# Nyrox/raymond

Measured on AMD Instinct MI355X. Metric: Msamples/s (whole node) + achieved HBM GB/s, 1920x1080 @ 500spp 5-bounce, higher is better.
Workload: dtype f64

## Files before the change

include/raymond_hip_probe.h:

```cpp
#ifndef RAYMOND_HIP_PROBE_H
#define RAYMOND_HIP_PROBE_H

#include "raymond_hip.h"

#ifdef __cplusplus
extern "C" {
#endif

rmd_status rmd_probe_philox4x32_10(rmd_context *ctx, size_t n, const uint32_t *ctr4, const uint32_t *key2, uint32_t *out4);
rmd_status rmd_probe_block_uniforms(rmd_context *ctx, uint64_t seed, size_t n, const uint32_t *pixel, const uint32_t *sample,
                                    const uint32_t *block, double *out5);
rmd_status rmd_probe_sphere_intersect(rmd_context *ctx, size_t n, const double *sphere4, const double *ray6, int32_t *hit, double *t);
rmd_status rmd_probe_sphere_normal(rmd_context *ctx, size_t n, const double *sphere4, const double *ray6, const double *t, double *n3);
rmd_status rmd_probe_plane_intersect(rmd_context *ctx, size_t n, const double *plane6, const double *ray6, int32_t *hit, double *t);
rmd_status rmd_probe_aabb_intersect(rmd_context *ctx, size_t n, const double *aabb6, const double *ray6, int32_t *hit, double *t);
rmd_status rmd_probe_triangle_intersect(rmd_context *ctx, size_t n, const double *pos9, const double *ray6, int32_t *hit, double *t);
rmd_status rmd_probe_triangle_normal(rmd_context *ctx, size_t n, const double *pos9, const double *nrm9, const double *ray6,
                                     const double *t, double *n3);
rmd_status rmd_probe_onb(rmd_context *ctx, size_t n, const double *n3, double *t3, double *b3);
rmd_status rmd_probe_cosine_hemisphere(rmd_context *ctx, size_t n, const double *r1, const double *r2, double *dir3, double *pdf);
rmd_status rmd_probe_importance_sample_ggx(rmd_context *ctx, size_t n, const double *reflect3, const double *rough, const double *r1,
                                           const double *r2, double *dir3);
rmd_status rmd_probe_ggx_distribution(rmd_context *ctx, size_t n, const double *n3, const double *h3, const double *rough, double *out);
rmd_status rmd_probe_geometry_smith(rmd_context *ctx, size_t n, const double *n3, const double *v3, const double *l3,
// ... 1 lines not shown
rmd_status rmd_probe_fresnel_schlick(rmd_context *ctx, size_t n, const double *cos_theta, const double *f0_3, double *out3);
rmd_status rmd_probe_elementary(rmd_context *ctx, size_t n, const double *x, double *sqrt_out, double *sin_out, double *cos_out,
                                double *root_out, double *inv_root_out);
rmd_status rmd_probe_primary_ray(rmd_context *ctx, size_t n, const rmd_camera *cam, const uint32_t *xy2, const double *u2, double *ray6);
rmd_status rmd_probe_scene_intersect(rmd_context *ctx, const rmd_scene *scene, size_t n, const double *ray6, int32_t *obj, double *t,
                                     uint32_t *sub);
rmd_status rmd_probe_grid_intersect(rmd_context *ctx, const rmd_scene *scene, uint32_t g, size_t n, const double *ray6, int32_t *hit,
                                    double *t, uint32_t *tri);
rmd_status rmd_probe_grid_intersect_deep(rmd_context *ctx, const rmd_scene *scene, uint32_t g, size_t n, const double *ray6, uint32_t cut_lanes,
                                         uint32_t cut_round, uint32_t rays_per_wave, int32_t *hit, double *t, uint32_t *tri);
rmd_status rmd_probe_trace_samples(rmd_context *ctx, const rmd_scene *scene, const rmd_camera *cam, const rmd_settings *settings,
                                   size_t n, const uint32_t *xy2, const uint32_t *sample, double *rgb_out, int32_t *path_obj,
                                   uint32_t *path_sub);

rmd_status rmd_probe_triangle_sphere(size_t n, const double *pos9, double *out5);
rmd_status rmd_probe_launch_plan(uint32_t mode, uint32_t grid, size_t n, const uint32_t *in5, uint64_t *out8);
rmd_status rmd_probe_launch_sizes(uint32_t mode, uint32_t grid, uint64_t *out8);
rmd_status rmd_probe_scene_layout(const rmd_scene *scene, uint32_t *n_objects, uint32_t *n_grids, uint32_t *mask_words_total);
rmd_status rmd_probe_pretest_pairs(rmd_context *ctx, size_t n, const double *sphere5, const double *pos9, const double *ray6, int32_t *pass,
                                   int32_t *hit, double *t);

#ifdef __cplusplus
}
#endif
#endif
```

raymond_amd/csrc/api.cpp:

```cpp
#define RMD_WITH_HIP 1
#include <algorithm>
#include <cmath>
#include <limits>
#include <cstdio>
#include <cstdlib>
#include <cstring>
#include <new>

#include "internal.hpp"
#include "launch.hpp"

namespace {
thread_local std::string tl_last_error;

rmd_status bind(rmd_context *ctx) {
	if (!ctx) return rmd::fail(nullptr, RMD_ERR_INVALID_ARGUMENT, "null context");
	RMD_HIP(ctx, hipSetDevice(ctx->device));
	return RMD_OK;
}

rmd_status context_create(int32_t device, hipStream_t stream, bool own_stream, rmd_context **out) {
	if (!out) return rmd::fail(nullptr, RMD_ERR_INVALID_ARGUMENT, "rmd_context_create: null out pointer");
	*out = nullptr;
	int count = 0;
// ... 137 lines not shown
	f[0] = 0u, f[1] = 0u, f[2] = 0u;
	std::string what;
	if (code & kFaultTripLoop) what += " trip loop of render_wave;";
	if (code & kFaultSortedTripLoop) what += " trip loop of render_wave_sorted;";
	if (code & kFaultWorkLoop) what += " work loop of a persistent workgroup;";
	if (code & kFaultWalkRounds) what += " round loop of a grid walk;";
	if (code & kFaultQueuedTripLoop) what += " trip loop of render_wave_queued;";
	if (code & ~(kFaultTripLoop | kFaultSortedTripLoop | kFaultWorkLoop | kFaultWalkRounds | kFaultQueuedTripLoop)) what += " unknown code;";
	char num[96];
	std::snprintf(num, sizeof(num), " %u wave(s) reported, the last one at work item %u (code 0x%x)", reports, item, code);
	return fail(ctx, RMD_ERR_DEVICE_FAULT,
	            "device fault: a loop of the render kernel ran past its bound —" + what + num +
	                "; the launch was cut short and the framebuffer it wrote to is not valid");
}

RenderParams make_params(const rmd_context *ctx, const rmd_scene *scene, const rmd_camera *cam, const rmd_settings *st) {
	const double PI = 3.14159265358979323846;
	RenderParams P;
	std::memset(&P, 0, sizeof(P));
	for (int a = 0; a < 3; a++) P.cam_pos[a] = cam->position[a];
	P.width = (double)cam->backbuffer_width;
	P.height = (double)cam->backbuffer_height;
	P.inv_width = rmd::exact_reciprocal(P.width), P.inv_height = rmd::exact_reciprocal(P.height);
	P.aspect = P.width / P.height;
	P.tan_half_fov = std::tan(cam->fov_vert / 2.0 * PI / 180.0);
	P.focal_length = cam->focal_length;
	P.aperture_radius = cam->aperture_radius;
	P.W = cam->backbuffer_width, P.H = cam->backbuffer_height;
	P.bounce_limit = st->bounce_limit;
	P.sample_begin = st->sample_begin, P.sample_count = st->sample_count;
	P.n_objects = scene ? scene->n_objects : 0;
	P.n_grids = scene ? scene->n_grids : 0;
	P.mask_words_total = scene ? scene->mask_words_total : 0;
	P.key0 = (uint32_t)st->seed, P.key1 = (uint32_t)(st->seed >> 32);
	P.use_dof = ((st->flags & RMD_RENDER_DOF) && cam->aperture_radius > 0.0) ? 1u : 0u;
	P.end_black_paths = (st->flags & RMD_RENDER_TRACE_BLACK_PATHS) ? 0u : ((st->flags & RMD_RENDER_END_BLACK_PATHS) || !scene || (scene->n_grids == 0u && scene->regular)) ? 1u : 0u;
	P.shade_last_depth = (scene && !scene->regular) ? 1u : 0u;
	P.axis_pairs = scene ? scene->axis_pairs : 0u;
	P.visit_mask = scene ? scene->visit_mask : ~0ull, P.grid_mask = scene ? scene->grid_mask : ~0ull;
	P.fault = ctx ? ctx->d_fault : nullptr;
	P.walk_batch = rmd::kWalkBatchDefault;
	if (ctx && ctx->tunable[RMD_TUNE_WALK_BATCH] > 0) P.walk_batch = (uint32_t)ctx->tunable[RMD_TUNE_WALK_BATCH];
	{
		uint32_t k = rmd::kWalkCutDefault;
		if (ctx && ctx->tunable[RMD_TUNE_WALK_CUT] > 0) k = (uint32_t)std::min<int64_t>(ctx->tunable[RMD_TUNE_WALK_CUT] - 1, 31);
		P.walk_cut = (scene && scene->n_grid_objects == 1u) ? (k | (2u * k) << 8) : 0u;
		P.walk_steps_bound = scene ? scene->walk_steps_bound : 0u;
	}
#if RMD_DIAG
	if (ctx) P.debug_flags = ctx->debug_flags;
#endif
	return P;
}

// ... 116 lines not shown
			}
		}
		out.aux.assign((size_t)g.n_tris * 4, 0.0);
		for (uint64_t ti = 0; ti < g.n_tris; ti++) rmd::triangle_aux(g.tri_pos + (size_t)ti * 9, out.aux.data() + (size_t)ti * 4);
		out.spheres.assign((size_t)g.n_tris * 4, 0.0);
		out.sphere_kb = 0.0;
		for (uint64_t ti = 0; ti < g.n_tris; ti++) {
			double kb = 0.0;
			rmd::triangle_sphere(g.tri_pos + (size_t)ti * 9, out.spheres.data() + (size_t)ti * 4, kb);
			out.sphere_kb = std::max(out.sphere_kb, kb);
		}
	}
	return RMD_OK;
}

static rmd_status scene_create_impl(rmd_context *ctx, const rmd_object *objects, uint32_t n_objects, const rmd_grid_desc *grids, uint32_t n_grids,
                                    rmd_scene **out) {
	if (rmd_status s = bind(ctx)) return s;
	if (!out || (n_objects && !objects) || (n_grids && !grids)) return rmd::fail(ctx, RMD_ERR_INVALID_ARGUMENT, "rmd_scene_create: null argument");
	std::vector<rmd::DevObject> hobj(n_objects);
	bool regular = true;
	for (uint32_t i = 0; i < n_objects; i++) {
		const rmd_object &o = objects[i];
		rmd::DevObject &d = hobj[i];
		std::memset(&d, 0, sizeof(d));
		if (o.geometry_kind > RMD_GEOM_GRID) return rmd::fail(ctx, RMD_ERR_INVALID_ARGUMENT, "rmd_scene_create: unknown geometry kind");
		if (o.material.kind > RMD_MAT_EMISSION) return rmd::fail(ctx, RMD_ERR_INVALID_ARGUMENT, "rmd_scene_create: unknown material kind");
		if (o.geometry_kind == RMD_GEOM_GRID && o.grid_index >= n_grids) return rmd::fail(ctx, RMD_ERR_INVALID_ARGUMENT, "rmd_scene_create: grid_index out of range");
		d.geometry_kind = o.geometry_kind, d.grid_index = o.grid_index, d.material_kind = o.material.kind;
		for (int a = 0; a < 3; a++) d.origin[a] = o.origin[a], d.normal[a] = o.normal[a], d.color[a] = o.material.color[a];
		d.radius = o.radius;
		if (o.material.kind != RMD_MAT_EMISSION && std::fabs(o.material.roughness) > rmd::kMaxRoughness)
			return rmd::fail(ctx, RMD_ERR_UNSUPPORTED, "rmd_scene_create: |roughness| > 512 is not supported");
		if (o.material.kind != RMD_MAT_EMISSION && o.material.roughness != 0.0 && std::fabs(o.material.roughness) < rmd::kMinRoughness)
			return rmd::fail(ctx, RMD_ERR_UNSUPPORTED, "rmd_scene_create: 0 < |roughness| < 1e-12 is not supported");
// ... 13 lines not shown
		}
		if (o.material.kind == RMD_MAT_DIFFUSE && o.material.color[0] == 0.0 && o.material.color[1] == 0.0 && o.material.color[2] == 0.0) d.flags |= rmd::kObjBlackDiffuse;
	}
	for (uint32_t j = 0; j < n_objects; j++) {
		if (hobj[j].geometry_kind != RMD_GEOM_PLANE) continue;
		for (uint32_t i = 0; i < j; i++) {
			if (hobj[i].geometry_kind != RMD_GEOM_PLANE || hobj[i].pair_info != 0u) continue;
			bool opposite = true;
			for (int a = 0; a < 3; a++) opposite = opposite && hobj[j].normal[a] == -hobj[i].normal[a];
			if (!opposite) continue;
			hobj[i].pair_info = rmd::kPairTestedAtPartner | j, hobj[j].pair_info = i + 1u;
			break;
		}
	}
	uint32_t axis_pairs = 0;
	for (uint32_t j = 0; j < n_objects && j < 1023u && regular && ctx->tunable[RMD_TUNE_AXIS_PAIRS] != 1; j++) {
		if (hobj[j].geometry_kind != RMD_GEOM_PLANE || hobj[j].pair_info == 0u || (hobj[j].pair_info & rmd::kPairTestedAtPartner)) continue;
		const uint32_t i = hobj[j].pair_info - 1u;
		int k = -1, nonzero = 0;
		for (int a = 0; a < 3; a++)
			if (hobj[i].normal[a] != 0.0) nonzero++, k = a;
		if (nonzero != 1 || (hobj[i].normal[k] != 1.0 && hobj[i].normal[k] != -1.0) || ((axis_pairs >> (10 * k)) & 1023u) != 0u) continue;
		axis_pairs |= (j + 1u) << (10 * k);
		hobj[j].flags |= rmd::kObjAxisPair | ((uint32_t)k << rmd::kObjAxisShift) | (hobj[i].normal[k] == 1.0 ? rmd::kObjAxisEarlierIsPlus : 0u);
		hobj[i].flags |= rmd::kObjAxisPair;
		hobj[j].partner_origin_k = hobj[i].origin[k];
		hobj[j].pair_info = rmd::kPairTestedAtPartner | rmd::kPairAxis | i;
		hobj[i].pair_info |= rmd::kPairAxis;
	}
	auto sc = std::make_unique<rmd_scene>();
	sc->ctx = ctx, sc->n_objects = n_objects, sc->n_grids = n_grids, sc->regular = regular;
	sc->axis_pairs = axis_pairs;
	rmd::DevObject walls_block;
	std::memset(&walls_block, 0, sizeof(walls_block));
	{
		rmd::AxisWalls walls[3];
		std::memset(walls, 0, sizeof(walls));
		for (int k = 0; k < 3; k++) {
			const uint32_t f = (axis_pairs >> (10 * k)) & 1023u;
			if (f == 0u) continue;
			const uint32_t j = f - 1u, i = hobj[j].pair_info & 0x3FFFFFFFu;
			const bool e_plus = (hobj[j].flags & rmd::kObjAxisEarlierIsPlus) != 0u;
			walls[k].o_plus = e_plus ? hobj[i].origin[k] : hobj[j].origin[k], walls[k].o_minus = e_plus ? hobj[j].origin[k] : hobj[i].origin[k];
			walls[k].idx_plus = e_plus ? i : j, walls[k].idx_minus = e_plus ? j : i;
		}
		std::memcpy(&walls_block, walls, sizeof(walls));
	}
	sc->visit_mask = 0ull, sc->grid_mask = 0ull;
	for (uint32_t i = 0; i < n_objects && i < 64u; i++) {
		if (!(hobj[i].geometry_kind == RMD_GEOM_PLANE && (hobj[i].pair_info & rmd::kPairTestedAtPartner))) sc->visit_mask |= 1ull << i;
		if (hobj[i].geometry_kind == RMD_GEOM_GRID) sc->grid_mask |= 1ull << i;
	}
	for (uint32_t i = 0; i < n_objects; i++) sc->n_grid_objects += objects[i].geometry_kind == RMD_GEOM_GRID ? 1u : 0u;
	auto upload = [&](const void *src, size_t bytes, void **dst) -> hipError_t {
		*dst = nullptr;
		rmd::DeviceBuffer b;
		hipError_t e = b.alloc(bytes ? bytes : 16);
		if (e != hipSuccess) return e;
		*dst = b.as<void>();
		sc->owned.push_back(std::move(b));
		if (bytes) e = hipMemcpy(*dst, src, bytes, hipMemcpyHostToDevice);
		return e;
	};
	std::vector<rmd::DevGrid> hgrid(n_grids);
	for (uint32_t gi = 0; gi < n_grids; gi++) {
		const rmd_grid_desc &g = grids[gi];
		rmd::DevGrid &d = hgrid[gi];
// ... 261 lines not shown
		if ((P.debug_flags & 16u) && ctx->last_launch.queued) {
			static const char *kinds[3] = {"GEN  ", "SHADE", "WALK "};
			for (int k = 0; k < 3; k++)
				std::fprintf(stderr, "[rmd queued stamps, cycles] %s trips=%llu fetch=%llu make_ray=%llu simple=%llu walk=%llu ray_push=%llu classify=%llu stores=%llu\n", kinds[k], h[k * 8 + 7],
				             h[k * 8 + 0], h[k * 8 + 1], h[k * 8 + 2], h[k * 8 + 3], h[k * 8 + 4], h[k * 8 + 5], h[k * 8 + 6]);
			std::fprintf(stderr, "[rmd queued stamps, cycles] inside the walks: init=%llu stepping=%llu entry_wait=%llu scan=%llu (chunk search+load+test)=%llu hits=%llu tail=%llu\n",
			             h[24], h[25], h[26], h[27], h[29], h[30], h[31]);
		} else if (P.debug_flags & 16u)
			std::fprintf(stderr, "[rmd stamps, cycles] wave_total=%llu next_ray=%llu simple=%llu walk=%llu classify=%llu | walk: init=%llu stepping=%llu entry_wait=%llu scan=%llu (chunk search+load+test)=%llu hits=%llu tail=%llu\n",
			             h[0], h[1], h[2], h[3], h[4], h[8], h[9], h[10], h[11], h[13], h[14], h[15]);
		else
			std::fprintf(stderr, "[rmd debug] walk_calls=%llu walkers=%llu calls_with_walkers=%llu rounds=%llu wave_steps=%llu lane_steps=%llu test_rounds=%llu tests=%llu chunks=%llu | main_iterations=%llu live_lanes=%llu lanes_with_ray=%llu | stepping iterations with <= 4 / 8 / 16 lanes: %llu / %llu / %llu, with <= 8 lanes while tests wait: %llu\n",
			             h[0], h[1], h[2], h[3], h[4], h[5], h[6], h[8], h[9], h[10], h[11], h[12], h[7], h[13], h[14], h[15]);
		if ((P.debug_flags & 16u) == 0u)
			std::fprintf(stderr, "[rmd debug] sphere pre-test: pairs passed=%llu full chunks=%llu | pairs dropped that pass the reference's test (flag 64; must be 0)=%llu\n", h[17], h[18], h[16]);
		if ((P.debug_flags & 16u) == 0u && ctx->last_launch.queued)
			std::fprintf(stderr, "[rmd debug] path queues: rays pushed=%llu (of them walks put aside=%llu) rays held in their lanes=%llu hits pushed=%llu hits held in their lanes=%llu\n", h[19], h[22], h[23], h[20], h[21]);
	}
	return RMD_OK;
}

rmd_status rmd_render_tiles_async(rmd_context *ctx, const rmd_scene *scene, const rmd_camera *camera, const rmd_settings *settings,
                                  const rmd_tile_rect *tiles, uint32_t n_tiles, double *accum_dev) {
	return rmd::guarded(ctx, "rmd_render_tiles", [&] { return render_tiles_async_impl(ctx, scene, camera, settings, tiles, n_tiles, accum_dev, nullptr); });
}

rmd_status rmd_render_tiles_moments_async(rmd_context *ctx, const rmd_scene *scene, const rmd_camera *camera, const rmd_settings *settings,
                                          const rmd_tile_rect *tiles, uint32_t n_tiles, double *accum_dev, double *accum_sq_dev) {
	if (accum_sq_dev != nullptr && accum_sq_dev == accum_dev)
		return rmd::fail(ctx, RMD_ERR_INVALID_ARGUMENT, "rmd_render_tiles_moments: accum_sq_dev must not alias accum_dev");
// ... 404 lines not shown
```

raymond_amd/csrc/device_types.hpp:

```cpp
#pragma once
#include <stdint.h>

namespace rmd {

struct alignas(16) DevObject {
	uint32_t geometry_kind;
	uint32_t grid_index;
	uint32_t material_kind;
	uint32_t pair_info;
	double origin[3];
	double radius;
	double normal[3];
	double roughness;
	double color[3];
	double metalness;
	uint32_t flags;
	uint32_t _pad2;
	double partner_origin_k;
};
constexpr uint32_t kObjBlackDiffuse = 1u;
constexpr uint32_t kObjAxisPair = 2u, kObjAxisShift = 8u, kObjAxisEarlierIsPlus = 1u << 10;
static_assert(sizeof(DevObject) == 128, "DevObject layout");
constexpr uint32_t kPairTestedAtPartner = 0x80000000u;
constexpr uint32_t kPairAxis = 0x40000000u;
// ... 57 lines not shown
	uint32_t n_work;
	uint32_t use_dof;
	uint32_t n_grids;
	uint32_t walk_batch;
	uint32_t mask_words_total;
	uint32_t split_k;
	double *sample_buf;
	uint32_t debug_flags;
	unsigned long long *debug_counters;
	uint32_t *work_counter;
	uint32_t *tile_done;
	uint32_t end_black_paths;
	uint32_t walk_cut;
	uint32_t shade_last_depth;
	uint32_t chain_items;
	uint32_t _pad1;
	uint32_t buffered;
	uint32_t axis_pairs;
	uint32_t _pad2;
	uint32_t *fault;
	unsigned char *queue_buf;
	uint32_t queue_wave_bytes;
	uint32_t queue_paths;
	uint32_t walk_steps_bound;
	uint32_t _pad3;
	unsigned long long visit_mask;
	unsigned long long grid_mask;
	unsigned long long sample_magic;
};
constexpr uint32_t kFaultTripLoop = 1u;
constexpr uint32_t kFaultSortedTripLoop = 2u;
// ... 12 lines not shown
```

raymond_amd/csrc/internal.hpp:

```cpp
#pragma once
#include <stdint.h>

#include <cmath>
#include <limits>
#include <algorithm>
#include <cstring>

#include <memory>
#include <mutex>
#include <string>
#include <vector>

#include "../../include/raymond_hip.h"

#ifdef RMD_WITH_HIP
#include <hip/hip_runtime_api.h>

#include "device_types.hpp"

#define RMD_HIP(ctx, call)                                                                                      \
	do {                                                                                                        \
		hipError_t e_ = (call);                                                                                 \
		if (e_ != hipSuccess) return rmd::fail(ctx, e_ == hipErrorOutOfMemory ? RMD_ERR_OUT_OF_MEMORY : RMD_ERR_HIP, \
		                                       std::string(#call) + ": " + hipGetErrorString(e_));              \
	} while (0)

namespace rmd {
class DeviceBuffer {
public:
	DeviceBuffer() = default;
	DeviceBuffer(DeviceBuffer &&o) noexcept : p_(o.p_), bytes_(o.bytes_) { o.p_ = nullptr, o.bytes_ = 0; }
	DeviceBuffer &operator=(DeviceBuffer &&o) noexcept {
		if (this != &o) (void)release(), p_ = o.p_, bytes_ = o.bytes_, o.p_ = nullptr, o.bytes_ = 0;
// ... 53 lines not shown
	hipStream_t copy_stream = nullptr;
	int64_t tunable[RMD_TUNE_COUNT] = {};
	uint32_t debug_flags = 0;
	rmd_launch_info last_launch = {};
	~rmd_context();
};

struct rmd_scene {
	rmd_context *ctx = nullptr;
	uint32_t n_objects = 0, n_grids = 0;
	uint32_t n_grid_objects = 0;
	uint32_t mask_words_total = 0;
	uint32_t axis_pairs = 0;
	unsigned long long visit_mask = ~0ull, grid_mask = ~0ull;
	uint32_t walk_steps_bound = 0;
	bool regular = true;
	rmd::DevObject *d_objects = nullptr;
	rmd::DevGrid *d_grids = nullptr;
	std::vector<rmd::DeviceBuffer> owned;
	~rmd_scene();
};
#endif

struct rmd_grid_build {
	double bbox_min[3], bbox_max[3], cell_size[3];
	uint32_t res[3];
	std::vector<uint32_t> cells, mapping;
	std::vector<double> pos, nrm;
	std::shared_ptr<void> derived;
	std::mutex derived_mutex;
// ... 66 lines not shown
template <class F>
rmd_status guarded(rmd_context *ctx, const char *what, F &&body) noexcept {
	try {
		return body();
	} catch (const std::bad_alloc &) {
		return fail_noexcept(ctx, RMD_ERR_OUT_OF_MEMORY, what, "the host ran out of memory");
	} catch (const std::exception &e) {
		return fail_noexcept(ctx, RMD_ERR_HIP, what, e.what());
	} catch (...) {
		return fail_noexcept(ctx, RMD_ERR_HIP, what, "unknown exception");
	}
}
#ifdef RMD_WITH_HIP
rmd_status check_fault(rmd_context *ctx);
RenderParams make_params(const rmd_context *ctx, const rmd_scene *scene, const rmd_camera *cam, const rmd_settings *st);
#endif
}
```

raymond_amd/csrc/probe.cpp:

```cpp
#define RMD_WITH_HIP 1
#include <cstring>
#include <vector>

#include "../../include/raymond_hip_probe.h"
#include "internal.hpp"
#include "launch.hpp"

namespace {

struct Column {
	const double *src;
	int width;
};

rmd_status run_probe(rmd_context *ctx, int op, size_t n, const std::vector<Column> &cols, int out_stride, std::vector<double> &out,
                     const rmd::RenderParams *params = nullptr) {
	if (!ctx) return rmd::fail(nullptr, RMD_ERR_INVALID_ARGUMENT, "probe: null context");
	RMD_HIP(ctx, hipSetDevice(ctx->device));
	int in_stride = 0;
	for (const Column &c : cols) {
		if (!c.src && n) return rmd::fail(ctx, RMD_ERR_INVALID_ARGUMENT, "probe: null input array");
		in_stride += c.width;
	}
	std::vector<double> in(n * in_stride);
// ... 202 lines not shown
	if (stuck) return rmd::fail(ctx, RMD_ERR_DEVICE_FAULT, "probe: a wave of the DEEP walk reached its bound of walk calls with rays unfinished (it cannot: an internal fault)");
	for (size_t i = 0; i < n; i++) hit[i] = (int32_t)out[3 * i], t[i] = out[3 * i + 1], tri[i] = (uint32_t)out[3 * i + 2];
	return RMD_OK;
}

rmd_status rmd_probe_triangle_sphere(size_t n, const double *pos9, double *out5) {
	if (n != 0 && (!pos9 || !out5)) return rmd::fail(nullptr, RMD_ERR_INVALID_ARGUMENT, "probe: bad argument");
	for (size_t i = 0; i < n; i++) {
		double kb = 0.0;
		rmd::triangle_sphere(pos9 + i * 9, out5 + i * 5, kb);
		out5[i * 5 + 4] = kb;
	}
	return RMD_OK;
}

rmd_status rmd_probe_launch_plan(uint32_t mode, uint32_t grid, size_t n, const uint32_t *in5, uint64_t *out8) {
	if (mode > 2u || grid > 1u || (n != 0 && (!in5 || !out8))) return rmd::fail(nullptr, RMD_ERR_INVALID_ARGUMENT, "probe: bad argument");
	for (size_t i = 0; i < n; i++) {
		const uint32_t *a = in5 + i * 5;
		const rmd::LaunchPlan L = rmd::plan_render_launch((int)mode, grid != 0u, a[0], a[1], (a[2] & 1u) != 0u, (a[2] & 2u) != 0u, (a[2] & 4u) != 0u,
		                                                  (a[2] & 8u) != 0u, a[3], a[4]);
		uint64_t *o = out8 + i * 8;
		o[0] = L.persistent, o[1] = L.queued, o[2] = L.chained, o[3] = L.moments, o[4] = L.waves_per_wg, o[5] = L.workgroups, o[6] = L.wave_lds, o[7] = L.lds;
	}
	return RMD_OK;
}

rmd_status rmd_probe_launch_sizes(uint32_t mode, uint32_t grid, uint64_t *out8) {
	if (mode > 2u || grid > 1u || !out8) return rmd::fail(nullptr, RMD_ERR_INVALID_ARGUMENT, "probe: bad argument");
	rmd::render_lds_sizes((int)mode, grid != 0u, out8);
// ... 56 lines not shown
```

raymond_amd/csrc/render_kernel.hpp:

```cpp
#pragma once
#include <hip/hip_runtime.h>

#include "device_core.hpp"
#include "grid_walk.hpp"
#include "launch.hpp"
#include "scene_split.hpp"

namespace rmd {

struct alignas(16) PathId {
	uint32_t px[64];
	uint32_t smp[64];
	uint32_t sector[64];
};
__host__ __device__ inline size_t wave_lds_bytes(uint32_t n_grids) { return kWaveHeadBytes + (n_grids ? sizeof(WalkScratch) + 64u * 3u * sizeof(double) + sizeof(WalkCarry) + sizeof(PathId) : 0); }

RMD_DEV uint32_t work_item_of_block(uint32_t b, uint32_t nb) {
	(void)nb;
	return b;
}

RMD_DEV void report_fault(const RenderParams &P, uint32_t code, uint32_t detail) {
	if ((threadIdx.x & 63u) == 0u) {
		if (P.fault != nullptr) {
// ... 492 lines not shown
		if constexpr (MOM && !acc_in_memory) out_sq[out_index + 0] = acc_sq.x, out_sq[out_index + 1] = acc_sq.y, out_sq[out_index + 2] = acc_sq.z;
	}
}

constexpr int kSortObjPrio = 1;
struct alignas(16) HitStack {
	double frag[3][kSortSlots], normal[3][kSortSlots], T[3][kSortSlots];
	uint32_t state[kSortSlots];
	uint32_t lobe_bits[kSortSlots];
	uint32_t item[kSortSlots];
};
static_assert(kSortSlots >= 72u && kSortSlots <= 512u && kSortSlots % 8u == 0u, "a generation trip needs room for 64 more hits");
static_assert(sizeof(HitStack) == kSortPoolBytes, "launch.hpp: kSortPoolBytes");
using SortPool = HitStack;

#define RMD_UNDEF3(v) RMD_UNDEF(v.x) RMD_UNDEF(v.y) RMD_UNDEF(v.z)
template <bool MOM = false>
RMD_DEV void render_wave_sorted(const RenderParams &P, KernargWords kernarg_params, const DevObject *__restrict__ objs, const DevGrid *__restrict__ grids,
                                const void *__restrict__ work, double *__restrict__ out, const DevObject *lobjs, unsigned char *wave_lds, uint32_t work_item,
                                double *__restrict__ out_sq = nullptr) {
	const uint32_t lane = threadIdx.x & 63u;
	HitStack &stack = *reinterpret_cast<HitStack *>(wave_lds);
	WalkScratch *no_scratch = nullptr;
	const uint32_t wt = work_item / P.split_k, part = work_item % P.split_k;
	const bool have = wt < P.n_work;
	const WaveTile tile = reinterpret_cast<const WaveTile *>(work)[have ? wt : 0];
	const uint32_t per_part = (P.sample_count + P.split_k - 1u) / P.split_k;
	const uint32_t s_lo = part * per_part < P.sample_count ? part * per_part : P.sample_count;
	const uint32_t s_hi = s_lo + per_part < P.sample_count ? s_lo + per_part : P.sample_count;
	const uint32_t pool_first = s_lo, pool_items = have ? (s_hi - s_lo) * 64u : 0u;
	if (P.bounce_limit == 0u) return;
	const V3 cam_pos = ld3(P.cam_pos);

	uint32_t n_hit = 0, next_item = 0;
	unsigned long long trips_left = (unsigned long long)pool_items * kTripBoundPerPair + 64ull;
#if RMD_DIAG
	if (P.debug_flags & 32u) trips_left = 1ull;
#endif
	for (;;) {
		KernargWords src = kernarg_params;
		asm volatile("" : "+s"(src));
		unsigned long long w[sizeof(RenderParams) / 8];
#pragma unroll
		for (unsigned i = 0; i < sizeof(RenderParams) / 8; i++) w[i] = src[i];
		RenderParams Pt;
		__builtin_memcpy(&Pt, w, sizeof(Pt));

		if (RMD_UNLIKELY(trips_left-- == 0ull)) {
			report_fault(Pt, kFaultSortedTripLoop, work_item);
			n_hit = 0u, next_item = pool_items;
		}
		const bool items_left = next_item < pool_items;
		if (n_hit == 0u && !items_left) break;
		const bool shade_trip = !items_left || n_hit > kSortSlots - 64u;
		bool active;
		uint32_t item = 0, depth = 1;
		Rng rng;
		rng.block = 0u, rng.lobe_bits = 0u;
		V3 ro, rd, T;
		RMD_UNDEF3(ro) RMD_UNDEF3(rd) RMD_UNDEF3(T)
		bool failed = false;
		if (shade_trip) {
			const uint32_t n = n_hit < 64u ? n_hit : 64u;
			active = lane < n;
			const uint32_t e = active ? n_hit - n + lane : 0u;
			n_hit -= n;
			const uint32_t st = stack.state[e];
			item = stack.item[e];
			const uint32_t lb = stack.lobe_bits[e];
			rng.block = st >> 16, rng.lobe_bits = lb & 0x3FFFFFu;
			depth = lb >> 24;
			const DevObject &o = lobjs[active ? (st & 0xFFFFu) : 0u];
			T = mk(stack.T[0][e], stack.T[1][e], stack.T[2][e]);
			const V3 normal = mk(stack.normal[0][e], stack.normal[1][e], stack.normal[2][e]);
			const V3 frag = mk(stack.frag[0][e], stack.frag[1][e], stack.frag[2][e]);
			const uint32_t x = tile.x0 + (item & 7u), y = tile.y0 + ((item >> 3) & 7u);
// ... 5 lines not shown
				failed = active && (depth > Pt.bounce_limit || black);
			}
		} else {
			item = next_item + lane;
			next_item += 64u;
			active = item < pool_items && (item & 7u) < tile.w && ((item >> 3) & 7u) < tile.h;
			const uint32_t x = tile.x0 + (item & 7u), y = tile.y0 + ((item >> 3) & 7u);
			rng.pixel = y * Pt.W + x, rng.sample = Pt.sample_begin + pool_first + (item >> 6);
			T = mk(1.0, 1.0, 1.0);
			{
				double u0, u1;
				rng.next2(Pt.key0, Pt.key1, u0, u1);
				primary_ray(Pt, x, y, u0, u1, ro, rd);
				if (Pt.use_dof) failed = active && !thin_lens_from_pinhole(Pt, ro, rd, rng, ro, rd);
			}
		}
		const bool want = active && !failed;
		double t = 0.0;
		uint32_t sub = 0;
		__builtin_amdgcn_s_setprio(kSortObjPrio);
		const int oi = scene_intersect_wave<false>(objs, Pt.n_objects, grids, nullptr, *no_scratch, want, ro, rd, t, sub, Pt.axis_pairs, 0u, nullptr, false, Pt.visit_mask);
		__builtin_amdgcn_s_setprio(0);
		bool terminal = failed, park = false, emitted = false;
		V3 frag, normal;
		RMD_UNDEF3(frag) RMD_UNDEF3(normal)
		if (want) {
			if (oi < 0) {
				terminal = true;
			} else {
				const DevObject &o = lobjs[oi];
				frag = ro + rd * t;
				if (o.material_kind == 2u) {
					emitted = true;
					terminal = true;
				} else {
					if (o.geometry_kind == 0u) normal = ld3(o.normal);
					else normal = normalize(frag - ld3(o.origin));
// ... 574 lines not shown
```

raymond_amd/probe.py:

```python
import ctypes as C
import os

import numpy as np

from . import abi
from . import lib as _lib

_vp = C.c_void_p
_sz = C.c_size_t
_P = C.POINTER
_SIGS = {
    "rmd_probe_philox4x32_10": [_vp, _sz, _vp, _vp, _vp],
    "rmd_probe_block_uniforms": [_vp, C.c_uint64, _sz, _vp, _vp, _vp, _vp],
    "rmd_probe_sphere_intersect": [_vp, _sz, _vp, _vp, _vp, _vp],
    "rmd_probe_sphere_normal": [_vp, _sz, _vp, _vp, _vp, _vp],
    "rmd_probe_plane_intersect": [_vp, _sz, _vp, _vp, _vp, _vp],
    "rmd_probe_aabb_intersect": [_vp, _sz, _vp, _vp, _vp, _vp],
    "rmd_probe_triangle_intersect": [_vp, _sz, _vp, _vp, _vp, _vp],
    "rmd_probe_triangle_normal": [_vp, _sz, _vp, _vp, _vp, _vp, _vp],
    "rmd_probe_onb": [_vp, _sz, _vp, _vp, _vp],
    "rmd_probe_cosine_hemisphere": [_vp, _sz, _vp, _vp, _vp, _vp],
    "rmd_probe_importance_sample_ggx": [_vp, _sz, _vp, _vp, _vp, _vp, _vp],
    "rmd_probe_ggx_distribution": [_vp, _sz, _vp, _vp, _vp, _vp],
    "rmd_probe_geometry_smith": [_vp, _sz, _vp, _vp, _vp, _vp, _vp],
    "rmd_probe_fresnel_schlick": [_vp, _sz, _vp, _vp, _vp],
    "rmd_probe_primary_ray": [_vp, _sz, _P(abi.Camera), _vp, _vp, _vp],
    "rmd_probe_elementary": [_vp, _sz, _vp, _vp, _vp, _vp, _vp, _vp],
    "rmd_probe_scene_intersect": [_vp, _vp, _sz, _vp, _vp, _vp, _vp],
    "rmd_probe_grid_intersect": [_vp, _vp, C.c_uint32, _sz, _vp, _vp, _vp, _vp],
    "rmd_probe_grid_intersect_deep": [_vp, _vp, C.c_uint32, _sz, _vp, C.c_uint32, C.c_uint32, C.c_uint32, _vp, _vp, _vp],
    "rmd_probe_trace_samples": [_vp, _vp, _P(abi.Camera), _P(abi.Settings), _sz, _vp, _vp, _vp, _vp, _vp],
    "rmd_probe_triangle_sphere": [_sz, _vp, _vp],
    "rmd_probe_pretest_pairs": [_vp, _sz, _vp, _vp, _vp, _vp, _vp, _vp],
    "rmd_probe_launch_plan": [C.c_uint32, C.c_uint32, _sz, _vp, _vp],
    "rmd_probe_launch_sizes": [C.c_uint32, C.c_uint32, _vp],
    "rmd_probe_scene_layout": [_vp, _P(C.c_uint32), _P(C.c_uint32), _P(C.c_uint32)],
}
PATH_STRIDE = 17
_ready = False


PROBE_LIB_PATH = os.path.join(os.path.dirname(_lib.LIB_PATH), "libraymond_hip_probe.so")
_probe_lib = None


def _L():
    global _ready, _probe_lib
    if not _ready:
# ... 129 lines not shown
    st = L.rmd_probe_triangle_sphere(pos9.shape[0], _p(pos9), _p(out))
    if st != _abi.RMD_OK:
        raise RuntimeError("rmd_probe_triangle_sphere: status %d" % st)
    return out[:, :3], out[:, 3], out[:, 4]


def pretest_pairs(ctx, sphere5, pos9, ray6):
    L = _L()
    sphere5, pos9, ray6 = _f(sphere5, 5), _f(pos9, 9), _f(ray6, 6)
    n = pos9.shape[0]
    passed, hit, t = np.zeros(n, dtype=np.int32), np.zeros(n, dtype=np.int32), np.zeros(n)
    ctx.check(L.rmd_probe_pretest_pairs(ctx.handle, n, _p(sphere5), _p(pos9), _p(ray6), _p(passed), _p(hit), _p(t)))
    return passed.astype(bool), hit.astype(bool), t


MODE_TILES, MODE_TILES_BUFFERED, MODE_LIST = 0, 1, 2
PLAN_QUEUES, PLAN_PERSIST, PLAN_CHAIN, PLAN_MOMENTS = 1, 2, 4, 8
PLAN_FIELDS = ("persistent", "queued", "chained", "moments", "waves_per_wg", "workgroups", "wave_lds", "lds")
SIZE_FIELDS = ("budget", "object", "wave", "queued_wave", "persist_waves", "grid_waves", "sort_pool", "mask_budget")


def _host_check(st, name):
    if st != abi.RMD_OK:
        raise RuntimeError("%s: status %d" % (name, st))


def launch_plan(mode, grid, n_objects, mask_words_total, flags, n_waves, n_cus):
    L = _L()
    cols = np.broadcast_arrays(*(np.asarray(a, dtype=np.int64) for a in (n_objects, mask_words_total, flags, n_waves, n_cus)))
    inp = np.ascontiguousarray(np.stack([c.ravel() for c in cols], axis=1).astype(np.uint32))
# ... 18 lines not shown
```

Baseline: 23400.

## Cull spheres and axis-wall pairs per wave tile for primary rays

For each 8x8 wave tile, the kernel builds a conservative cone around the tile's primary rays. Spheres that lie entirely outside that cone are dropped from the visit mask, and axis-wall pairs that cannot be the closest hit are trimmed. The reduced sets are used in the primary-ray scene intersection of render_wave_sorted, which skips intersection tests that cannot hit. The cost is extra per-item cone math and LDS traffic. Correctness depends on the conservative margins, and the cull is only enabled for regular scenes without grids or depth of field.

```diff
diff --git a/include/raymond_hip_probe.h b/include/raymond_hip_probe.h
--- a/include/raymond_hip_probe.h
+++ b/include/raymond_hip_probe.h
@@ -39,6 +39,8 @@
                                    uint32_t *path_sub);
 
 rmd_status rmd_probe_triangle_sphere(size_t n, const double *pos9, double *out5);
+rmd_status rmd_probe_primary_candidates(const rmd_camera *cam, const rmd_settings *settings, const rmd_object *objects, uint32_t n_objects, uint32_t n_grids,
+                                        int64_t axis_pairs_tunable, size_t n_tiles, const uint32_t *tiles4, uint64_t *launch3, uint64_t *out2);
 rmd_status rmd_probe_launch_plan(uint32_t mode, uint32_t grid, size_t n, const uint32_t *in5, uint64_t *out8);
 rmd_status rmd_probe_launch_sizes(uint32_t mode, uint32_t grid, uint64_t *out8);
 rmd_status rmd_probe_scene_layout(const rmd_scene *scene, uint32_t *n_objects, uint32_t *n_grids, uint32_t *mask_words_total);
diff --git a/raymond_amd/csrc/api.cpp b/raymond_amd/csrc/api.cpp
--- a/raymond_amd/csrc/api.cpp
+++ b/raymond_amd/csrc/api.cpp
@@ -175,6 +175,13 @@
 	                "; the launch was cut short and the framebuffer it wrote to is not valid");
 }
 
+bool primary_cull_allowed(const RenderParams &P) {
+	CullCamera c;
+	for (int a = 0; a < 3; a++) c.pos[a] = P.cam_pos[a];
+	c.width = P.width, c.height = P.height, c.aspect = P.aspect, c.tan_half_fov = P.tan_half_fov;
+	return P.use_dof == 0u && cull_camera_ok(c);
+}
+
 RenderParams make_params(const rmd_context *ctx, const rmd_scene *scene, const rmd_camera *cam, const rmd_settings *st) {
 	const double PI = 3.14159265358979323846;
 	RenderParams P;
@@ -199,6 +206,7 @@
 	P.shade_last_depth = (scene && !scene->regular) ? 1u : 0u;
 	P.axis_pairs = scene ? scene->axis_pairs : 0u;
 	P.visit_mask = scene ? scene->visit_mask : ~0ull, P.grid_mask = scene ? scene->grid_mask : ~0ull;
+	P.primary_cull = (scene && scene->primary_cull && rmd::primary_cull_allowed(P)) ? 1u : 0u;
 	P.fault = ctx ? ctx->d_fault : nullptr;
 	P.walk_batch = rmd::kWalkBatchDefault;
 	if (ctx && ctx->tunable[RMD_TUNE_WALK_BATCH] > 0) P.walk_batch = (uint32_t)ctx->tunable[RMD_TUNE_WALK_BATCH];
@@ -345,11 +353,9 @@
 	return RMD_OK;
 }
 
-static rmd_status scene_create_impl(rmd_context *ctx, const rmd_object *objects, uint32_t n_objects, const rmd_grid_desc *grids, uint32_t n_grids,
-                                    rmd_scene **out) {
-	if (rmd_status s = bind(ctx)) return s;
-	if (!out || (n_objects && !objects) || (n_grids && !grids)) return rmd::fail(ctx, RMD_ERR_INVALID_ARGUMENT, "rmd_scene_create: null argument");
-	std::vector<rmd::DevObject> hobj(n_objects);
+extern "C++" rmd_status rmd::derive_scene_objects(rmd_context *ctx, const rmd_object *objects, uint32_t n_objects, uint32_t n_grids, int64_t axis_pairs_tunable, rmd::SceneObjects &out) {
+	std::vector<rmd::DevObject> &hobj = out.objs;
+	hobj.assign(n_objects, rmd::DevObject{});
 	bool regular = true;
 	for (uint32_t i = 0; i < n_objects; i++) {
 		const rmd_object &o = objects[i];
@@ -393,7 +399,7 @@
 		}
 	}
 	uint32_t axis_pairs = 0;
-	for (uint32_t j = 0; j < n_objects && j < 1023u && regular && ctx->tunable[RMD_TUNE_AXIS_PAIRS] != 1; j++) {
+	for (uint32_t j = 0; j < n_objects && j < 1023u && regular && axis_pairs_tunable != 1; j++) {
 		if (hobj[j].geometry_kind != RMD_GEOM_PLANE || hobj[j].pair_info == 0u || (hobj[j].pair_info & rmd::kPairTestedAtPartner)) continue;
 		const uint32_t i = hobj[j].pair_info - 1u;
 		int k = -1, nonzero = 0;
@@ -407,14 +413,9 @@
 		hobj[j].pair_info = rmd::kPairTestedAtPartner | rmd::kPairAxis | i;
 		hobj[i].pair_info |= rmd::kPairAxis;
 	}
-	auto sc = std::make_unique<rmd_scene>();
-	sc->ctx = ctx, sc->n_objects = n_objects, sc->n_grids = n_grids, sc->regular = regular;
-	sc->axis_pairs = axis_pairs;
-	rmd::DevObject walls_block;
-	std::memset(&walls_block, 0, sizeof(walls_block));
 	{
-		rmd::AxisWalls walls[3];
-		std::memset(walls, 0, sizeof(walls));
+		rmd::AxisWalls *walls = out.walls;
+		std::memset(walls, 0, 3 * sizeof(rmd::AxisWalls));
 		for (int k = 0; k < 3; k++) {
 			const uint32_t f = (axis_pairs >> (10 * k)) & 1023u;
 			if (f == 0u) continue;
@@ -423,13 +424,33 @@
 			walls[k].o_plus = e_plus ? hobj[i].origin[k] : hobj[j].origin[k], walls[k].o_minus = e_plus ? hobj[j].origin[k] : hobj[i].origin[k];
 			walls[k].idx_plus = e_plus ? i : j, walls[k].idx_minus = e_plus ? j : i;
 		}
-		std::memcpy(&walls_block, walls, sizeof(walls));
-	}
-	sc->visit_mask = 0ull, sc->grid_mask = 0ull;
+	}
+	out.visit_mask = 0ull, out.grid_mask = 0ull;
 	for (uint32_t i = 0; i < n_objects && i < 64u; i++) {
-		if (!(hobj[i].geometry_kind == RMD_GEOM_PLANE && (hobj[i].pair_info & rmd::kPairTestedAtPartner))) sc->visit_mask |= 1ull << i;
-		if (hobj[i].geometry_kind == RMD_GEOM_GRID) sc->grid_mask |= 1ull << i;
-	}
+		if (!(hobj[i].geometry_kind == RMD_GEOM_PLANE && (hobj[i].pair_info & rmd::kPairTestedAtPartner))) out.visit_mask |= 1ull << i;
+		if (hobj[i].geometry_kind == RMD_GEOM_GRID) out.grid_mask |= 1ull << i;
+	}
+	out.regular = regular, out.axis_pairs = axis_pairs;
+	return RMD_OK;
+}
+
+static rmd_status scene_create_impl(rmd_context *ctx, const rmd_object *objects, uint32_t n_objects, const rmd_grid_desc *grids, uint32_t n_grids,
+                                    rmd_scene **out) {
+	if (rmd_status s = bind(ctx)) return s;
+	if (!out || (n_objects && !objects) || (n_grids && !grids)) return rmd::fail(ctx, RMD_ERR_INVALID_ARGUMENT, "rmd_scene_create: null argument");
+	rmd::SceneObjects derived;
+	if (rmd_status s = rmd::derive_scene_objects(ctx, objects, n_objects, n_grids, ctx->tunable[RMD_TUNE_AXIS_PAIRS], derived)) return s;
+	std::vector<rmd::DevObject> &hobj = derived.objs;
+	const bool regular = derived.regular;
+	const uint32_t axis_pairs = derived.axis_pairs;
+	auto sc = std::make_unique<rmd_scene>();
+	sc->ctx = ctx, sc->n_objects = n_objects, sc->n_grids = n_grids, sc->regular = regular;
+	sc->axis_pairs = axis_pairs;
+	rmd::DevObject walls_block;
+	std::memset(&walls_block, 0, sizeof(walls_block));
+	std::memcpy(&walls_block, derived.walls, sizeof(derived.walls));
+	sc->visit_mask = derived.visit_mask, sc->grid_mask = derived.grid_mask;
+	sc->primary_cull = regular && n_grids == 0u && ctx->tunable[RMD_TUNE_AXIS_PAIRS] == 0;
 	for (uint32_t i = 0; i < n_objects; i++) sc->n_grid_objects += objects[i].geometry_kind == RMD_GEOM_GRID ? 1u : 0u;
 	auto upload = [&](const void *src, size_t bytes, void **dst) -> hipError_t {
 		*dst = nullptr;
@@ -721,6 +742,9 @@
 			             h[0], h[1], h[2], h[3], h[4], h[5], h[6], h[8], h[9], h[10], h[11], h[12], h[7], h[13], h[14], h[15]);
 		if ((P.debug_flags & 16u) == 0u)
 			std::fprintf(stderr, "[rmd debug] sphere pre-test: pairs passed=%llu full chunks=%llu | pairs dropped that pass the reference's test (flag 64; must be 0)=%llu\n", h[17], h[18], h[16]);
+		if ((P.debug_flags & 16u) == 0u && (P.debug_flags & 512u))
+			std::fprintf(stderr, "[rmd debug] primary candidates: lanes checked=%llu sphere turns left out=%llu trips with two axis pairs left out=%llu | cleared spheres that register a hit (must be 0)=%llu closest hits that differ from the full visit's (must be 0)=%llu\n",
+			             h[32], h[35], h[36], h[33], h[34]);
 		if ((P.debug_flags & 16u) == 0u && ctx->last_launch.queued)
 			std::fprintf(stderr, "[rmd debug] path queues: rays pushed=%llu (of them walks put aside=%llu) rays held in their lanes=%llu hits pushed=%llu hits held in their lanes=%llu\n", h[19], h[22], h[23], h[20], h[21]);
 	}
diff --git a/raymond_amd/csrc/device_types.hpp b/raymond_amd/csrc/device_types.hpp
--- a/raymond_amd/csrc/device_types.hpp
+++ b/raymond_amd/csrc/device_types.hpp
@@ -95,7 +95,7 @@
 	uint32_t walk_cut;
 	uint32_t shade_last_depth;
 	uint32_t chain_items;
-	uint32_t _pad1;
+	uint32_t primary_cull;
 	uint32_t buffered;
 	uint32_t axis_pairs;
 	uint32_t _pad2;
diff --git a/raymond_amd/csrc/internal.hpp b/raymond_amd/csrc/internal.hpp
--- a/raymond_amd/csrc/internal.hpp
+++ b/raymond_amd/csrc/internal.hpp
@@ -17,6 +17,7 @@
 #include <hip/hip_runtime_api.h>
 
 #include "device_types.hpp"
+#include "primary_candidates.hpp"
 
 #define RMD_HIP(ctx, call)                                                                                      \
 	do {                                                                                                        \
@@ -100,6 +101,7 @@
 	uint32_t axis_pairs = 0;
 	unsigned long long visit_mask = ~0ull, grid_mask = ~0ull;
 	uint32_t walk_steps_bound = 0;
+	bool primary_cull = false;
 	bool regular = true;
 	rmd::DevObject *d_objects = nullptr;
 	rmd::DevGrid *d_grids = nullptr;
@@ -196,5 +198,14 @@
 #ifdef RMD_WITH_HIP
 rmd_status check_fault(rmd_context *ctx);
 RenderParams make_params(const rmd_context *ctx, const rmd_scene *scene, const rmd_camera *cam, const rmd_settings *st);
+bool primary_cull_allowed(const RenderParams &P);
+struct SceneObjects {
+	std::vector<DevObject> objs;
+	bool regular = true;
+	uint32_t axis_pairs = 0;
+	AxisWalls walls[3] = {};
+	unsigned long long visit_mask = 0ull, grid_mask = 0ull;
+};
+rmd_status derive_scene_objects(rmd_context *ctx, const rmd_object *objects, uint32_t n_objects, uint32_t n_grids, int64_t axis_pairs_tunable, SceneObjects &out);
 #endif
 }
diff --git a/raymond_amd/csrc/primary_candidates.hpp b/raymond_amd/csrc/primary_candidates.hpp
--- /dev/null
+++ b/raymond_amd/csrc/primary_candidates.hpp
@@ -0,0 +1,113 @@
+#pragma once
+#include <stdint.h>
+
+#include "device_types.hpp"
+
+#if defined(__HIP__)
+#define RMD_HD __host__ __device__ inline
+#else
+#define RMD_HD inline
+#endif
+
+namespace rmd {
+
+constexpr double kCullWiden = 1e-9;
+constexpr double kCullSphereMargin = 3200.0 * 2.220446049250313e-16;
+constexpr double kCullFacing = 2e-6;
+constexpr double kCullPairMargin = 1e-9;
+
+struct CullCamera {
+	double pos[3];
+	double width, height, aspect, tan_half_fov;
+};
+struct TileCone {
+	double lo[2], hi[2];
+	double a[3];
+	double cos_t, sin_t;
+	double u_max;
+	bool ok;
+};
+RMD_HD double cull_abs(double v) { return v < 0.0 ? -v : v; }
+RMD_HD double cull_min(double a, double b) { return a < b ? a : b; }
+RMD_HD double cull_max(double a, double b) { return a > b ? a : b; }
+
+RMD_HD bool cull_camera_ok(const CullCamera &c) {
+	const double big = 1e150;
+	bool ok = cull_abs(c.pos[0]) <= big && cull_abs(c.pos[1]) <= big && cull_abs(c.pos[2]) <= big;
+	ok = ok && c.tan_half_fov > 0.0 && c.tan_half_fov <= big && c.aspect > 0.0 && c.aspect <= big;
+	return ok && c.width > 0.0 && c.width <= big && c.height > 0.0 && c.height <= big;
+}
+
+RMD_HD TileCone primary_tile_cone(const CullCamera &c, uint32_t x0, uint32_t y0, uint32_t w, uint32_t h) {
+	TileCone T;
+	const double ex = c.tan_half_fov * c.aspect, ey = c.tan_half_fov;
+	const double pxa = (2.0 * ((double)x0 / c.width) - 1.0) * ex, pxb = (2.0 * ((double)(x0 + w) / c.width) - 1.0) * ex;
+	const double pya = (1.0 - 2.0 * ((double)y0 / c.height)) * ey, pyb = (1.0 - 2.0 * ((double)(y0 + h) / c.height)) * ey;
+	T.lo[0] = cull_min(pxa, pxb) - kCullWiden * ex, T.hi[0] = cull_max(pxa, pxb) + kCullWiden * ex;
+	T.lo[1] = cull_min(pya, pyb) - kCullWiden * ey, T.hi[1] = cull_max(pya, pyb) + kCullWiden * ey;
+	const double cx = 0.5 * (T.lo[0] + T.hi[0]), cy = 0.5 * (T.lo[1] + T.hi[1]);
+	const double cl = __builtin_sqrt((cx * cx + cy * cy) + 1.0);
+	T.a[0] = cx / cl, T.a[1] = cy / cl, T.a[2] = 1.0 / cl;
+	double cos_t = 1.0, sin_t = 0.0, u_max = 1.0;
+	for (int k = 0; k < 4; k++) {
+		const double qx = (k & 1) ? T.hi[0] : T.lo[0], qy = (k & 2) ? T.hi[1] : T.lo[1];
+		const double ql = __builtin_sqrt((qx * qx + qy * qy) + 1.0);
+		const double dx = qx / ql, dy = qy / ql, dz = 1.0 / ql;
+		const double cs = (T.a[0] * dx + T.a[1] * dy) + T.a[2] * dz;
+		const double kx = T.a[1] * dz - T.a[2] * dy, ky = T.a[2] * dx - T.a[0] * dz, kz = T.a[0] * dy - T.a[1] * dx;
+		const double sn = __builtin_sqrt((kx * kx + ky * ky) + kz * kz);
+		cos_t = cull_min(cos_t, cs), sin_t = cull_max(sin_t, sn), u_max = cull_max(u_max, ql);
+	}
+	T.cos_t = cos_t, T.sin_t = sin_t, T.u_max = u_max;
+	T.ok = cos_t > 0.7072 && sin_t < 0.7072 && u_max < 1e150 && T.lo[0] > -1e150 && T.hi[0] < 1e150 && T.lo[1] > -1e150 && T.hi[1] < 1e150;
+	return T;
+}
+
+RMD_HD bool primary_sphere_cleared(const TileCone &T, const CullCamera &c, const double centre[3], double radius) {
+	if (!T.ok) return false;
+	const double vx = centre[0] - c.pos[0], vy = centre[1] - c.pos[1], vz = centre[2] - c.pos[2];
+	const double va = (vx * T.a[0] + vy * T.a[1]) + vz * T.a[2];
+	const double kx = vy * T.a[2] - vz * T.a[1], ky = vz * T.a[0] - vx * T.a[2], kz = vx * T.a[1] - vy * T.a[0];
+	const double vxa = __builtin_sqrt((kx * kx + ky * ky) + kz * kz);
+	const double r = cull_abs(radius);
+	const double K = ((cull_abs(vx) + cull_abs(vy)) + cull_abs(vz)) + ((cull_abs(centre[0]) + cull_abs(centre[1])) + cull_abs(centre[2])) +
+	                 ((cull_abs(c.pos[0]) + cull_abs(c.pos[1])) + cull_abs(c.pos[2])) + r;
+	const double margin = kCullSphereMargin * K;
+	const bool in_front = va * T.cos_t - vxa * T.sin_t > margin;
+	const double D = vxa * T.cos_t - va * T.sin_t;
+	return in_front && D > r + margin && K <= 1e150;
+}
+
+RMD_HD uint32_t primary_pairs_kept(const TileCone &T, const CullCamera &c, const AxisWalls walls[3], uint32_t axis_pairs) {
+	if (!T.ok) return axis_pairs;
+	double s_lo[3], s_hi[3];
+	bool paired[3];
+	for (int k = 0; k < 3; k++) {
+		paired[k] = ((axis_pairs >> (10 * k)) & 1023u) != 0u;
+		s_lo[k] = 0.0, s_hi[k] = -1.0;
+		if (!paired[k]) continue;
+		const double num_plus = c.pos[k] - walls[k].o_plus, num_minus = walls[k].o_minus - c.pos[k];
+		if (!(num_plus > 0.0 && num_minus > 0.0)) return axis_pairs;
+		const double lo = k < 2 ? T.lo[k] : 1.0, hi = k < 2 ? T.hi[k] : 1.0;
+		double nearest = 1e300;
+		if (hi > 0.0) nearest = cull_min(nearest, num_minus / hi);
+		if (lo < 0.0) nearest = cull_min(nearest, num_plus / -lo);
+		s_lo[k] = nearest;
+		if (!(s_lo[k] > 0.0)) return axis_pairs;
+		const bool pos = lo > 0.0, neg = hi < 0.0;
+		if (pos || neg) {
+			const double u_lo = pos ? lo : -hi;
+			if (u_lo > kCullFacing * T.u_max) s_hi[k] = (pos ? num_minus : num_plus) / u_lo;
+		}
+	}
+	for (int k = 0; k < 3; k++) {
+		if (!paired[k] || !(s_hi[k] > 0.0)) continue;
+		bool alone = true;
+		for (int j = 0; j < 3; j++)
+			if (j != k && paired[j]) alone = alone && s_hi[k] * (1.0 + kCullPairMargin) < s_lo[j];
+		if (alone) return axis_pairs & (1023u << (10 * k));
+	}
+	return axis_pairs;
+}
+
+}
diff --git a/raymond_amd/csrc/probe.cpp b/raymond_amd/csrc/probe.cpp
--- a/raymond_amd/csrc/probe.cpp
+++ b/raymond_amd/csrc/probe.cpp
@@ -240,6 +240,35 @@
 	return RMD_OK;
 }
 
+rmd_status rmd_probe_primary_candidates(const rmd_camera *cam, const rmd_settings *settings, const rmd_object *objects, uint32_t n_objects, uint32_t n_grids,
+                                        int64_t axis_pairs_tunable, size_t n_tiles, const uint32_t *tiles4, uint64_t *launch3, uint64_t *out2) {
+	if (!cam || !settings || (n_objects && !objects) || !launch3 || (n_tiles != 0 && (!tiles4 || !out2))) return rmd::fail(nullptr, RMD_ERR_INVALID_ARGUMENT, "probe: bad argument");
+	return rmd::guarded(nullptr, "rmd_probe_primary_candidates", [&]() -> rmd_status {
+		rmd::SceneObjects sc;
+		if (rmd_status s = rmd::derive_scene_objects(nullptr, objects, n_objects, n_grids, axis_pairs_tunable, sc)) return s;
+		const rmd::RenderParams P = rmd::make_params(nullptr, nullptr, cam, settings);
+		const bool on = sc.regular && n_grids == 0u && axis_pairs_tunable == 0 && rmd::primary_cull_allowed(P);
+		launch3[0] = sc.visit_mask, launch3[1] = sc.axis_pairs, launch3[2] = on ? 1u : 0u;
+		rmd::CullCamera cc;
+		for (int a = 0; a < 3; a++) cc.pos[a] = P.cam_pos[a];
+		cc.width = P.width, cc.height = P.height, cc.aspect = P.aspect, cc.tan_half_fov = P.tan_half_fov;
+		for (size_t i = 0; i < n_tiles; i++) {
+			const uint32_t *t = tiles4 + i * 4;
+			uint64_t visit = sc.visit_mask;
+			uint32_t pairs = sc.axis_pairs;
+			if (on) {
+				if (t[2] == 0u || t[2] > 8u || t[3] == 0u || t[3] > 8u || t[0] > 65535u || t[1] > 65535u) return rmd::fail(nullptr, RMD_ERR_INVALID_ARGUMENT, "probe: a wave tile is 1..8 pixels a side");
+				const rmd::TileCone cone = rmd::primary_tile_cone(cc, t[0], t[1], t[2], t[3]);
+				for (uint32_t j = 0; j < n_objects && j < 64u; j++)
+					if (sc.objs[j].geometry_kind == 1u && rmd::primary_sphere_cleared(cone, cc, sc.objs[j].origin, sc.objs[j].radius)) visit &= ~(1ull << j);
+				pairs = rmd::primary_pairs_kept(cone, cc, sc.walls, sc.axis_pairs);
+			}
+			out2[i * 2] = visit, out2[i * 2 + 1] = pairs;
+		}
+		return RMD_OK;
+	});
+}
+
 rmd_status rmd_probe_launch_plan(uint32_t mode, uint32_t grid, size_t n, const uint32_t *in5, uint64_t *out8) {
 	if (mode > 2u || grid > 1u || (n != 0 && (!in5 || !out8))) return rmd::fail(nullptr, RMD_ERR_INVALID_ARGUMENT, "probe: bad argument");
 	for (size_t i = 0; i < n; i++) {
diff --git a/raymond_amd/csrc/render_kernel.hpp b/raymond_amd/csrc/render_kernel.hpp
--- a/raymond_amd/csrc/render_kernel.hpp
+++ b/raymond_amd/csrc/render_kernel.hpp
@@ -4,6 +4,7 @@
 #include "device_core.hpp"
 #include "grid_walk.hpp"
 #include "launch.hpp"
+#include "primary_candidates.hpp"
 #include "scene_split.hpp"
 
 namespace rmd {
@@ -530,6 +531,35 @@
 static_assert(sizeof(HitStack) == kSortPoolBytes, "launch.hpp: kSortPoolBytes");
 using SortPool = HitStack;
 
+RMD_DEV void item_candidates(KernargWords kernarg_params, WaveTile tile, const DevObject *__restrict__ objs, const DevObject *lobjs, uint32_t *sets) {
+	const uint32_t lane = threadIdx.x & 63u;
+	KernargWords src = kernarg_params;
+	asm volatile("" : "+s"(src));
+	unsigned long long w[sizeof(RenderParams) / 8];
+#pragma unroll
+	for (unsigned i = 0; i < sizeof(RenderParams) / 8; i++) w[i] = src[i];
+	RenderParams P;
+	__builtin_memcpy(&P, w, sizeof(P));
+	unsigned long long visit = P.visit_mask;
+	uint32_t pairs = P.axis_pairs;
+	if (P.primary_cull != 0u) {
+		CullCamera cc;
+		cc.pos[0] = P.cam_pos[0], cc.pos[1] = P.cam_pos[1], cc.pos[2] = P.cam_pos[2];
+		cc.width = P.width, cc.height = P.height, cc.aspect = P.aspect, cc.tan_half_fov = P.tan_half_fov;
+		const TileCone cone = primary_tile_cone(cc, tile.x0, tile.y0, tile.w, tile.h);
+		const DevObject &o = lobjs[lane < P.n_objects ? lane : 0u];
+		const double centre[3] = {o.origin[0], o.origin[1], o.origin[2]};
+		const bool cleared = lane < P.n_objects && o.geometry_kind == 1u && primary_sphere_cleared(cone, cc, centre, o.radius);
+		visit &= ~__ballot(cleared);
+		const AxisWalls *walls = reinterpret_cast<const AxisWalls *>(objs + P.n_objects);
+		const AxisWalls w3[3] = {walls[0], walls[1], walls[2]};
+		pairs = primary_pairs_kept(cone, cc, w3, P.axis_pairs);
+	}
+	if (lane == 0u) sets[0] = pairs, sets[1] = (uint32_t)visit, sets[2] = (uint32_t)(visit >> 32);
+	__builtin_amdgcn_fence(__ATOMIC_RELEASE, "wavefront");
+	__builtin_amdgcn_wave_barrier();
+	__builtin_amdgcn_fence(__ATOMIC_ACQUIRE, "wavefront");
+}
 #define RMD_UNDEF3(v) RMD_UNDEF(v.x) RMD_UNDEF(v.y) RMD_UNDEF(v.z)
 template <bool MOM = false>
 RMD_DEV void render_wave_sorted(const RenderParams &P, KernargWords kernarg_params, const DevObject *__restrict__ objs, const DevGrid *__restrict__ grids,
@@ -548,6 +578,9 @@
 	if (P.bounce_limit == 0u) return;
 	const V3 cam_pos = ld3(P.cam_pos);
 
+	uint32_t *item_sets = reinterpret_cast<uint32_t *>(wave_lds + sizeof(HitStack)) + 1;
+	item_candidates(kernarg_params, tile, objs, lobjs, item_sets);
+
 	uint32_t n_hit = 0, next_item = 0;
 	unsigned long long trips_left = (unsigned long long)pool_items * kTripBoundPerPair + 64ull;
 #if RMD_DIAG
@@ -576,6 +609,8 @@
 		V3 ro, rd, T;
 		RMD_UNDEF3(ro) RMD_UNDEF3(rd) RMD_UNDEF3(T)
 		bool failed = false;
+		unsigned long long turns = Pt.visit_mask;
+		uint32_t pairs = Pt.axis_pairs;
 		if (shade_trip) {
 			const uint32_t n = n_hit < 64u ? n_hit : 64u;
 			active = lane < n;
@@ -611,13 +646,36 @@
 				primary_ray(Pt, x, y, u0, u1, ro, rd);
 				if (Pt.use_dof) failed = active && !thin_lens_from_pinhole(Pt, ro, rd, rng, ro, rd);
 			}
+			pairs = (uint32_t)__builtin_amdgcn_readfirstlane((int)item_sets[0]);
+			turns = (unsigned long long)(uint32_t)__builtin_amdgcn_readfirstlane((int)item_sets[1]) | (unsigned long long)(uint32_t)__builtin_amdgcn_readfirstlane((int)item_sets[2]) << 32;
 		}
 		const bool want = active && !failed;
 		double t = 0.0;
 		uint32_t sub = 0;
 		__builtin_amdgcn_s_setprio(kSortObjPrio);
-		const int oi = scene_intersect_wave<false>(objs, Pt.n_objects, grids, nullptr, *no_scratch, want, ro, rd, t, sub, Pt.axis_pairs, 0u, nullptr, false, Pt.visit_mask);
+		const int oi = scene_intersect_wave<false>(objs, Pt.n_objects, grids, nullptr, *no_scratch, want, ro, rd, t, sub, pairs, 0u, nullptr, false, turns);
 		__builtin_amdgcn_s_setprio(0);
+#if RMD_DIAG
+		if ((Pt.debug_flags & 512u) && (Pt.debug_flags & 8u) && Pt.debug_counters && !shade_trip) {
+			double t_full = 0.0;
+			uint32_t sub_full = 0;
+			const int oi_full = scene_intersect_wave<false>(objs, Pt.n_objects, grids, nullptr, *no_scratch, want, ro, rd, t_full, sub_full, Pt.axis_pairs, 0u, nullptr, false, Pt.visit_mask);
+			const bool differs = want && (oi_full != oi || __builtin_bit_cast(unsigned long long, t_full) != __builtin_bit_cast(unsigned long long, t));
+			unsigned long long wrong = 0ull;
+			const unsigned long long dropped = Pt.visit_mask & ~turns;
+			for (unsigned long long m = dropped; m != 0ull; m &= m - 1ull) {
+				const DevObject &o = objs[__builtin_ctzll(m)];
+				double ts;
+				wrong += (unsigned long long)__popcll(__ballot(want && sphere_test_flat(ld3(o.origin), o.radius, ro, rd, ts)));
+			}
+			const unsigned long long dm = __ballot(differs), wm = __ballot(want);
+			if (lane == 0u) {
+				atomicAdd(&Pt.debug_counters[32], (unsigned long long)__popcll(wm)), atomicAdd(&Pt.debug_counters[33], wrong);
+				atomicAdd(&Pt.debug_counters[34], (unsigned long long)__popcll(dm)), atomicAdd(&Pt.debug_counters[35], (unsigned long long)__popcll(dropped));
+				atomicAdd(&Pt.debug_counters[36], pairs != Pt.axis_pairs ? 1ull : 0ull);
+			}
+		}
+#endif
 		bool terminal = failed, park = false, emitted = false;
 		V3 frag, normal;
 		RMD_UNDEF3(frag) RMD_UNDEF3(normal)
diff --git a/raymond_amd/probe.py b/raymond_amd/probe.py
--- a/raymond_amd/probe.py
+++ b/raymond_amd/probe.py
@@ -32,6 +32,7 @@
     "rmd_probe_trace_samples": [_vp, _vp, _P(abi.Camera), _P(abi.Settings), _sz, _vp, _vp, _vp, _vp, _vp],
     "rmd_probe_triangle_sphere": [_sz, _vp, _vp],
     "rmd_probe_pretest_pairs": [_vp, _sz, _vp, _vp, _vp, _vp, _vp, _vp],
+    "rmd_probe_primary_candidates": [_P(abi.Camera), _P(abi.Settings), _P(abi.Object), C.c_uint32, C.c_uint32, C.c_int64, _sz, _vp, _vp, _vp],
     "rmd_probe_launch_plan": [C.c_uint32, C.c_uint32, _sz, _vp, _vp],
     "rmd_probe_launch_sizes": [C.c_uint32, C.c_uint32, _vp],
     "rmd_probe_scene_layout": [_vp, _P(C.c_uint32), _P(C.c_uint32), _P(C.c_uint32)],
@@ -191,6 +192,19 @@
     return passed.astype(bool), hit.astype(bool), t
 
 
+def primary_candidates(cam, settings, scene, tiles, axis_pairs_tunable=0):
+    L = _L()
+    objs, n, _descs, ng, keep = scene.flatten()
+    tiles = np.ascontiguousarray(tiles, dtype=np.uint32).reshape(-1, 4)
+    launch, out = np.zeros(3, dtype=np.uint64), np.zeros((tiles.shape[0], 2), dtype=np.uint64)
+    c, s = cam.pod(), settings.pod()
+    st = L.rmd_probe_primary_candidates(C.byref(c), C.byref(s), objs, n, ng, int(axis_pairs_tunable), tiles.shape[0], _p(tiles), _p(launch), _p(out))
+    del keep
+    if st != abi.RMD_OK:
+        raise RuntimeError("rmd_probe_primary_candidates: status %d" % st)
+    return int(launch[0]), int(launch[1]), bool(launch[2]), out[:, 0].copy(), out[:, 1].astype(np.uint32)
+
+
 MODE_TILES, MODE_TILES_BUFFERED, MODE_LIST = 0, 1, 2
 PLAN_QUEUES, PLAN_PERSIST, PLAN_CHAIN, PLAN_MOMENTS = 1, 2, 4, 8
 PLAN_FIELDS = ("persistent", "queued", "chained", "moments", "waves_per_wg", "workgroups", "wave_lds", "lds")
```

New measurement: 25190 (median of 6 runs). 1.08x the previous value.
